# mlrun/mlrun

Measured on NVIDIA H100. Metric: events/sec, higher is better.
Workload: dtype f32 in / f64 accumulate

## Files before the change

mlrun_b200/csrc/b2s_rowthread.cuh:

```cuda
#pragma once
#include <cuda.h>
#include <type_traits>

#include "b2s_device.cuh"
#include "b2s_hash.cuh"

namespace b2s {

constexpr int kRTMaxCatCols = 16;
constexpr int kRTCatsInline = 4;
constexpr int kRTMaxCats = 256;

template <int NCH, int NS>
struct RTParams {
  const char* rows;
  int64_t row_stride;
  int64_t n_rows;
  float* out;
  int32_t* status;
  int32_t n_in, out_cols, n_models, vote_kind, out_is_int, fast_epilogue, tile_rows, pitch, stages, vec_ok;
  int32_t n_cat_cols, n_cat;
  int32_t one_sync;
  int32_t use_bulk;
  float* peers[8];
  int64_t peer_off;
  int32_t n_peers;
  MergeSig sig;
  const double* wcat;
  const double* vote_w_g;
  const ModelDesc* models;
  const int32_t* classes;
  double w[NCH * 4][NS];
  float fill[NCH * 4];
  float lim[NCH * 4];
  double bias[NS];
  double vote_w[NS];
  int32_t cat_col[kRTMaxCatCols];
  int32_t cat_off[kRTMaxCatCols];
  int32_t cat_sw[kRTMaxCatCols];
  int32_t cat_base[kRTMaxCatCols];
  int32_t cat_cnt[kRTMaxCatCols];
  float cat_fill[kRTMaxCatCols];
  float cat_inl[kRTMaxCatCols][kRTCatsInline];
  int32_t cat_first[kRTMaxCatCols];
  int32_t cat_dense[kRTMaxCatCols];
  float cat_val[kRTMaxCats];
  struct CatFast {
    int32_t off_b;
    int32_t sw_b;
    int32_t first;
    int32_t cnt;
    int32_t woff_b;
    float fill;
    int32_t pad[2];
  };
  CatFast catf[kRTMaxCatCols];
  int32_t cats_fast;
  int32_t zero_woff_b;
  int32_t dead_tail;
  int32_t pad_fast;
  const long long* g_keys;
  const TableSlot* g_slots;
  uint64_t g_mask;
  const float* g_values;
  long long g_missing_row;
};

struct RowPadded {
  const float* xr;
  __device__ __forceinline__ float4 chunk(int ch) const { return *reinterpret_cast<const float4*>(xr + ch * 4); }
  __device__ __forceinline__ float at2(int off, int) const { return xr[off]; }
  __device__ __forceinline__ float at_b(int off_b, int) const { return *reinterpret_cast<const float*>(reinterpret_cast<const char*>(xr) + off_b); }
};
struct RowSwizzled {
  const float* box0;
  int box_words;
  int r7s;
  __device__ __forceinline__ float4 chunk(int ch) const {
    return *reinterpret_cast<const float4*>(box0 + (ch >> 3) * box_words + (((ch & 7) << 2) ^ r7s));
  }
  __device__ __forceinline__ float at2(int off, int sw) const { return box0[off + (sw ^ r7s)]; }
  __device__ __forceinline__ float at_b(int off_b, int sw_b) const {
    return *reinterpret_cast<const float*>(reinterpret_cast<const char*>(box0) + off_b + (sw_b ^ (r7s << 2)));
  }
};

template <int NCH, int NS, int CH0, int CH1, typename Row>
__device__ __forceinline__ void rt_slice(const RTParams<NCH, NS>& p, const Row (&xr)[1], double (&acc)[1][NS]) {
  constexpr int RPT = 1;
  constexpr int BATCH = 4;
#pragma unroll
  for (int b = CH0; b < CH1; b += BATCH) {
    double xd[RPT][BATCH * 4];
#pragma unroll
    for (int cb = 0; cb < BATCH; ++cb) {
      const int ch = b + cb;
      if (ch < CH1) {
#pragma unroll
        for (int i = 0; i < RPT; ++i) {
          const float4 v = xr[i].chunk(ch);
          const float xs[4] = {v.x, v.y, v.z, v.w};
#pragma unroll
          for (int u = 0; u < 4; ++u) {
            const int c = ch * 4 + u;
            float x = xs[u];
            x = !(fabsf(x) <= p.lim[c]) ? p.fill[c] : x;
            xd[i][cb * 4 + u] = (double)x;
          }
        }
      }
    }
#pragma unroll
    for (int cb = 0; cb < BATCH; ++cb) {
      const int ch = b + cb;
      if (ch < CH1) {
#pragma unroll
        for (int u = 0; u < 4; ++u) {
          const int c = ch * 4 + u;
#pragma unroll
          for (int k = 0; k < NS; ++k)
#pragma unroll
            for (int i = 0; i < RPT; ++i) acc[i][k] = fma(p.w[c][k], xd[i][cb * 4 + u], acc[i][k]);
        }
      }
    }
  }
}

template <int NCH, int NS>
__device__ __noinline__ int rt_cat_search(const RTParams<NCH, NS>& p, int cc, float x) {
  const int b0 = p.cat_base[cc], cnt = p.cat_cnt[cc];
  int j = p.n_cat;
  if (cnt <= kRTCatsInline) {
#pragma unroll
    for (int qq = kRTCatsInline - 1; qq >= 0; --qq) j = (x == p.cat_inl[cc][qq]) ? b0 + qq : j;
  } else {
    for (int qq = cnt - 1; qq >= 0; --qq) j = (x == p.cat_val[b0 + qq]) ? b0 + qq : j;
  }
  return j;
}

template <int NCH, int NS, int Q0, int TPR, typename Row>
__device__ __forceinline__ void rt_cats(const RTParams<NCH, NS>& p, const Row (&xr)[1], const double* __restrict__ s_wcat,
                                        double (&acc)[1][NS]) {
  constexpr int RPT = 1;
  constexpr int ITERS = (kRTMaxCatCols - Q0 + TPR - 1) / TPR;
  if (p.cats_fast) {
    const char* wb = reinterpret_cast<const char*>(s_wcat);
#pragma unroll
    for (int it = 0; it < ITERS; ++it) {
      const int cc = Q0 + it * TPR;
      if (cc >= p.n_cat_cols) break;
      const typename RTParams<NCH, NS>::CatFast cf = p.catf[cc];
#pragma unroll
      for (int i = 0; i < RPT; ++i) {
        float x = xr[i].at_b(cf.off_b, cf.sw_b);
        x = (x != x) ? cf.fill : x;
        const int v = __float2int_rz(x);
        const unsigned jj = (unsigned)(v - cf.first);
        const bool miss = ((float)v != x) | (jj >= (unsigned)cf.cnt);
        const int a = miss ? p.zero_woff_b : cf.woff_b + (int)jj * (NS * 8);
        if constexpr (NS % 2 == 0) {
#pragma unroll
          for (int k = 0; k < NS; k += 2) {
            const double2 w2 = *reinterpret_cast<const double2*>(wb + a + k * 8);
            acc[i][k] += w2.x;
            acc[i][k + 1] += w2.y;
          }
        } else {
          const double* wc = reinterpret_cast<const double*>(wb + a);
#pragma unroll
          for (int k = 0; k < NS; ++k) acc[i][k] += wc[k];
        }
      }
    }
    return;
  }
#pragma unroll
  for (int it = 0; it < ITERS; ++it) {
    const int cc = Q0 + it * TPR;
    if (cc >= p.n_cat_cols) break;
#pragma unroll
    for (int i = 0; i < RPT; ++i) {
      float x = xr[i].at2(p.cat_off[cc], p.cat_sw[cc]);
      x = (x != x) ? p.cat_fill[cc] : x;
      int j;
      if (p.cat_dense[cc]) {
        const int v = __float2int_rz(x);
        const unsigned jj = (unsigned)(v - p.cat_first[cc]);
        j = ((float)v == x && jj < (unsigned)p.cat_cnt[cc]) ? p.cat_base[cc] + (int)jj : p.n_cat;
      } else {
        j = rt_cat_search(p, cc, x);
      }
      const double* wc = s_wcat + (size_t)j * NS;
#pragma unroll
      for (int k = 0; k < NS; ++k) acc[i][k] += wc[k];
    }
  }
}

template <int NCH, int NS, int TPR, int LIVE, typename Row>
__device__ __forceinline__ void rt_row_slices(const RTParams<NCH, NS>& p, int q, const Row (&xr)[1], const double* __restrict__ s_wcat,
                                              double (&acc)[1][NS]) {
  static_assert(LIVE % TPR == 0, "live chunks must split evenly over the row's threads");
  constexpr int CPT = LIVE / TPR;
  if (TPR == 1 || q == 0) {
    rt_slice<NCH, NS, 0, CPT>(p, xr, acc);
    rt_cats<NCH, NS, 0, TPR>(p, xr, s_wcat, acc);
  } else if (q == 1) {
    rt_slice<NCH, NS, (TPR > 1 ? CPT : 0), (TPR > 1 ? 2 * CPT : 0)>(p, xr, acc);
    rt_cats<NCH, NS, (TPR > 1 ? 1 : 0), TPR>(p, xr, s_wcat, acc);
  } else if (q == 2) {
    rt_slice<NCH, NS, (TPR > 2 ? 2 * CPT : 0), (TPR > 2 ? 3 * CPT : 0)>(p, xr, acc);
    rt_cats<NCH, NS, (TPR > 2 ? 2 : 0), TPR>(p, xr, s_wcat, acc);
  } else {
    rt_slice<NCH, NS, (TPR > 3 ? 3 * CPT : 0), (TPR > 3 ? 4 * CPT : 0)>(p, xr, acc);
    rt_cats<NCH, NS, (TPR > 3 ? 3 : 0), TPR>(p, xr, s_wcat, acc);
  }
}

__device__ __forceinline__ void mbar_init(uint64_t* bar, int count) {
  asm volatile("mbarrier.init.shared::cta.b64 [%0], %1;" ::"r"((uint32_t)__cvta_generic_to_shared(bar)), "r"(count));
}
__device__ __forceinline__ void mbar_expect_tx(uint64_t* bar, uint32_t bytes) {
  asm volatile("mbarrier.arrive.expect_tx.shared::cta.b64 _, [%0], %1;" ::"r"((uint32_t)__cvta_generic_to_shared(bar)), "r"(bytes)
               : "memory");
}
__device__ __forceinline__ void mbar_wait(uint64_t* bar, uint32_t parity) {
  const uint32_t a = (uint32_t)__cvta_generic_to_shared(bar);
  asm volatile(
      "{\n"
      ".reg .pred p;\n"
      "WAIT_%=:\n"
      "mbarrier.try_wait.parity.shared::cta.b64 p, [%0], %1;\n"
      "@p bra DONE_%=;\n"
      "bra WAIT_%=;\n"
      "DONE_%=:\n"
      "}\n" ::"r"(a), "r"(parity)
      : "memory");
}
__device__ __forceinline__ void bulk_load(void* smem_dst, const void* gsrc, uint32_t bytes, uint64_t* bar) {
  asm volatile("cp.async.bulk.shared::cluster.global.mbarrier::complete_tx::bytes [%0], [%1], %2, [%3];" ::"r"(
                   (uint32_t)__cvta_generic_to_shared(smem_dst)),
               "l"(gsrc), "r"(bytes), "r"((uint32_t)__cvta_generic_to_shared(bar))
               : "memory");
}

__device__ __forceinline__ void tensor_load_2d(void* smem_dst, const CUtensorMap* tmap, int x, int y, uint64_t* bar) {
  asm volatile(
      "cp.async.bulk.tensor.2d.shared::cluster.global.tile.mbarrier::complete_tx::bytes [%0], [%1, {%2, %3}], [%4];" ::"r"(
          (uint32_t)__cvta_generic_to_shared(smem_dst)),
      "l"(reinterpret_cast<uint64_t>(tmap)), "r"(x), "r"(y), "r"((uint32_t)__cvta_generic_to_shared(bar))
      : "memory");
}

template <int NCH, int NS>
__device__ __noinline__ void rt_generic_epilogue(const RTParams<NCH, NS>& p, const double* sl, int64_t row, uint32_t st) {
  double pred[kMaxModels];
  for (int m = 0; m < p.n_models; ++m) {
    const ModelDesc md = p.models[m];
    pred[m] = apply_link(md, sl + md.score_off, p.classes);
  }
  KParams kp;
  kp.out = p.out;
  kp.out_cols = p.out_cols;
  kp.n_models = p.n_models;
  kp.vote_kind = p.vote_kind;
  kp.out_is_int = p.out_is_int;
  kp.vote_w = p.vote_w_g;
  kp.status = p.status;
  kp.n_peers = p.n_peers;
  kp.peer_off = p.peer_off;
  for (int g = 0; g < p.n_peers; ++g) kp.peers[g] = p.peers[g];
  vote_and_store(kp, pred, row, st);
}

template <int NCH, int NS, int TPR, int LM>
__global__ void __launch_bounds__(128 * TPR, TPR >= 4 ? 2 : (TPR == 2 ? 3 : 4))
    rowthread_kernel(const __grid_constant__ RTParams<NCH, NS> p, const __grid_constant__ CUtensorMap tmap) {
  constexpr int RPT = 1;
  static_assert(NCH % TPR == 0, "chunks must split evenly over the row's threads");
  constexpr int CPT = NCH / TPR;
  extern __shared__ __align__(16) unsigned char smem[];
  uint64_t* s_bar = reinterpret_cast<uint64_t*>(smem);
  double* s_wcat = reinterpret_cast<double*>(smem + 64);
  const size_t wcat_bytes = 64 + (((size_t)(p.n_cat + 1) * NS * 8 + 15) / 16) * 16;
  const bool one_sync = (LM == 2) && TPR > 1 && p.one_sync;
  constexpr size_t part_words = (size_t)(TPR - 1) * 128 * NS;
  double* s_part = reinterpret_cast<double*>(smem + wcat_bytes);
  float* s_tiles = reinterpret_cast<float*>(smem + wcat_bytes + (one_sync ? 2 : 1) * part_words * 8);
  if (LM == 2) {
    const uint32_t a = (uint32_t)__cvta_generic_to_shared(s_tiles);
    s_tiles += ((1024u - (a & 1023u)) & 1023u) >> 2;
  }

  const int tid = threadIdx.x;
  const int TR = p.tile_rows;
  const int S = p.stages;
  const int tile_words = (LM == 2) ? TR * NCH * 4 : TR * p.pitch;
  const int64_t n_tiles = (p.n_rows + TR - 1) / TR;
  const int TRT = TR / RPT;
  const int q = tid / TRT;
  const int r = tid - q * TRT;

  const int cprv = p.vec_ok ? (p.n_in >> 2) : p.n_in;
  const int r0 = tid / cprv, c0 = tid - r0 * cprv;
  const int dr = (int)blockDim.x / cprv, dc = (int)blockDim.x - dr * cprv;
  auto issue = [&](float* tile, int64_t row0) {
    int64_t left = p.n_rows - row0;
    const int rows = left < TR ? (left < 0 ? 0 : (int)left) : TR;
    const char* base = p.rows + row0 * p.row_stride;
    int rr = r0, cc = c0;
    if (p.vec_ok) {
      while (rr < rows) {
        cp_async16(tile + rr * p.pitch + cc * 4, base + (int64_t)rr * p.row_stride + cc * 16);
        rr += dr;
        cc += dc;
        if (cc >= cprv) {
          cc -= cprv;
          ++rr;
        }
      }
    } else {
      while (rr < rows) {
        cp_async4(tile + rr * p.pitch + cc, base + (int64_t)rr * p.row_stride + cc * 4);
        rr += dr;
        cc += dc;
        if (cc >= cprv) {
          cc -= cprv;
          ++rr;
        }
      }
    }
  };

  constexpr bool bulk = LM != 0;
  const uint32_t row_bytes = (uint32_t)p.n_in * 4u;
  uint32_t unknown_bits = 0;
  long long gk_cur = 0, gk_nxt = 0;
  longlong2 g_slot = make_longlong2(0, -1);
  uint64_t g_hash = 0;
  int64_t g_tile_nxt = 0;
  auto g_key = [&](int64_t tile) -> long long {
    const int64_t row = tile * TR + tid;
    return row < p.n_rows ? __ldg(p.g_keys + row) : 0;
  };
  auto g_probe_start = [&](long long key) {
    g_hash = mix64((uint64_t)key) & p.g_mask;
    g_slot = __ldg(reinterpret_cast<const longlong2*>(p.g_slots) + g_hash);
  };
  auto g_probe_finish = [&](long long key) -> long long {
    uint64_t h = g_hash;
    longlong2 sl = g_slot;
    for (;;) {
      if (sl.y < 0) return -1;
      if (sl.x == key) return sl.y;
      h = (h + 1) & p.g_mask;
      sl = __ldg(reinterpret_cast<const longlong2*>(p.g_slots) + h);
    }
  };
  if (LM == 1 && p.g_keys && tid < TR) {
    gk_cur = g_key(blockIdx.x);
    gk_nxt = g_key((int64_t)blockIdx.x + gridDim.x);
    g_probe_start(gk_cur);
    g_tile_nxt = (int64_t)blockIdx.x + 2 * (int64_t)gridDim.x;
  }
  auto issue_bulk = [&](int st, int64_t row0) {
    int64_t left = p.n_rows - row0;
    const int rows = left < TR ? (left < 0 ? 0 : (int)left) : TR;
    if (LM == 2) {
      if (tid == 0) {
        if (rows > 0) {
          mbar_expect_tx(&s_bar[st], (uint32_t)(NCH / 8) * (uint32_t)TR * 128u);
#pragma unroll
          for (int b = 0; b < NCH / 8; ++b)
            tensor_load_2d(s_tiles + st * tile_words + b * TR * 32, &tmap, b * 32, (int)row0, &s_bar[st]);
        } else {
          mbar_expect_tx(&s_bar[st], 0);
        }
      }
    } else {
      if (tid == 0) mbar_expect_tx(&s_bar[st], (uint32_t)rows * row_bytes);
      if (p.g_keys) {
        if (tid < TR) {
          const long long hit = g_probe_finish(gk_cur);
          if (tid < rows) {
            unknown_bits = (unknown_bits & ~(1u << st)) | ((hit < 0 ? 1u : 0u) << st);
            bulk_load(s_tiles + st * tile_words + tid * p.pitch,
                      reinterpret_cast<const char*>(p.g_values + (hit < 0 ? p.g_missing_row : hit) * p.n_in), row_bytes, &s_bar[st]);
          }
          gk_cur = gk_nxt;
          g_probe_start(gk_cur);
          gk_nxt = g_key(g_tile_nxt);
          g_tile_nxt += gridDim.x;
        }
      } else if (tid < rows) {
        bulk_load(s_tiles + st * tile_words + tid * p.pitch, p.rows + (row0 + tid) * p.row_stride, row_bytes, &s_bar[st]);
      }
    }
  };
  if (bulk) {
    if (tid == 0) {
      for (int s = 0; s < S; ++s) mbar_init(&s_bar[s], 1);
      asm volatile("fence.mbarrier_init.release.cluster;" ::: "memory");
    }
    __syncthreads();
  }
  for (int s = 0; s < (one_sync ? S : S - 1); ++s) {
    const int64_t t = (int64_t)blockIdx.x + (int64_t)s * gridDim.x;
    if (bulk) {
      issue_bulk(s, t * TR);
    } else {
      if (t < n_tiles) issue(s_tiles + s * tile_words, t * TR);
      cp_async_commit();
    }
  }
  uint32_t phase_bits = 0;
  for (int i = tid; i < p.n_cat * NS; i += blockDim.x) s_wcat[i] = p.wcat[i];
  for (int i = tid; i < NS; i += blockDim.x) s_wcat[p.n_cat * NS + i] = 0.0;
  if (one_sync) __syncthreads();

  int stage = 0;
  uint32_t iter = 0;
  for (int64_t t = blockIdx.x; t < n_tiles; t += gridDim.x) {
    if (bulk) {
      mbar_wait(&s_bar[stage], (phase_bits >> stage) & 1u);
      phase_bits ^= (1u << stage);
    } else if (S == 2) cp_async_wait<0>();
    else if (S == 3) cp_async_wait<1>();
    else cp_async_wait<2>();
    if (!one_sync) {
      __syncthreads();
      const int64_t tn = t + (int64_t)(S - 1) * gridDim.x;
      int sn = stage + S - 1;
      if (sn >= S) sn -= S;
      if (bulk) {
        issue_bulk(sn, tn * TR);
      } else {
        if (tn < n_tiles) issue(s_tiles + sn * tile_words, tn * TR);
        cp_async_commit();
      }
    }
    const float* tile = s_tiles + stage * tile_words;
    const int64_t row0 = t * TR;
    const int live_rows = (int)(p.n_rows - row0 < (int64_t)TR ? p.n_rows - row0 : (int64_t)TR);
    const bool any_live = r < live_rows;
    using Row = typename std::conditional<LM == 2, RowSwizzled, RowPadded>::type;
    Row xr[RPT];
#pragma unroll
    for (int i = 0; i < RPT; ++i) {
      const int ri = r + i * TRT;
      if constexpr (LM == 2) {
        xr[i].box0 = tile + ri * 32;
        xr[i].box_words = TR * 32;
        xr[i].r7s = (r & 7) << 2;
      } else {
        xr[i].xr = tile + ri * p.pitch;
      }
    }
    double acc[RPT][NS];
#pragma unroll
    for (int i = 0; i < RPT; ++i)
#pragma unroll
      for (int k = 0; k < NS; ++k) acc[i][k] = 0.0;
    if (any_live) {
      if constexpr (LM == 2 && RPT == 1 && NCH >= 8 && (TPR == 1 || TPR == 2)) {
        if (p.dead_tail >= 4) rt_row_slices<NCH, NS, TPR, NCH - 4>(p, q, xr, s_wcat, acc);
        else if (p.dead_tail >= 2) rt_row_slices<NCH, NS, TPR, NCH - 2>(p, q, xr, s_wcat, acc);
        else rt_row_slices<NCH, NS, TPR, NCH>(p, q, xr, s_wcat, acc);
      } else {
        rt_row_slices<NCH, NS, TPR, NCH>(p, q, xr, s_wcat, acc);
      }
    }
    if (TPR > 1) {
      double* s_part_cur = s_part + (one_sync ? (size_t)(iter & 1) * part_words : 0);
      if (q > 0) {
#pragma unroll
        for (int i = 0; i < RPT; ++i) {
          double* part = s_part_cur + ((size_t)(q - 1) * 128 + r + i * TRT) * NS;
#pragma unroll
          for (int k = 0; k < NS; ++k) part[k] = acc[i][k];
        }
      }
      __syncthreads();
      if (one_sync) issue_bulk(stage, (t + (int64_t)S * gridDim.x) * TR);
      if (q == 0) {
#pragma unroll
        for (int i = 0; i < RPT; ++i)
#pragma unroll
          for (int qq = 1; qq < TPR; ++qq) {
            const double* o = s_part_cur + ((size_t)(qq - 1) * 128 + r + i * TRT) * NS;
#pragma unroll
            for (int k = 0; k < NS; ++k) acc[i][k] += o[k];
          }
      }
    }
#pragma unroll
    for (int i = 0; i < RPT; ++i) {
      const int64_t row = row0 + (r + i * TRT);
      if (q == 0 && r + i * TRT < live_rows) {
        uint32_t st = 0;
#pragma unroll
        for (int k = 0; k < NS; ++k) {
          acc[i][k] += p.bias[k];
          st |= (fabs(acc[i][k]) <= 1.7976931348623157e308) ? 0u : 1u;
        }
        if (LM == 1) st |= ((unknown_bits >> stage) & 1u) << 2;
        if (p.fast_epilogue) {
          if (p.vote_kind == 1) {
            double s = 0.0;
#pragma unroll
            for (int k = 0; k < NS; ++k) s = __dadd_rn(s, __dmul_rn(acc[i][k], p.vote_w[k]));
            store_word(p, row, 0, __float_as_uint((float)s));
          } else {
#pragma unroll
            for (int k = 0; k < NS; ++k)
              if (k < p.n_models) store_word(p, row, k, __float_as_uint((float)acc[i][k]));
          }
          if (p.status) p.status[row] = (int32_t)st;
        } else {
          double sl[NS];
#pragma unroll
          for (int k = 0; k < NS; ++k) sl[k] = acc[i][k];
          rt_generic_epilogue(p, sl, row, st);
        }
      }
    }
    ++stage;
    ++iter;
    if (stage == S) stage = 0;
  }
  cp_async_wait<0>();
  merge_signal(p.sig);
}

}
```

mlrun_b200/csrc/b2s_runtime.cu:

```cuda
#include <cuda_runtime.h>

#include <exception>

#include <algorithm>
#include <atomic>
#include <chrono>
#include <cmath>
#include <condition_variable>
#include <cstdarg>
#include <cstdio>
#include <cstdlib>
#include <cstring>
#include <deque>
#include <limits>
#include <map>
#include <memory>
#include <mutex>
#include <string>
#include <thread>
#include <vector>

#include "../../include/b200serve.h"
#include "b2s_internal.h"
#include "b2s_device.cuh"
// ... 181 lines not shown

int b2s_int_plan_shape(b2s_plan_s* p, int* n_in, int* out_cols) {
  if (!p || !p->finalized) return fail(B2S_ERR_STATE, "plan not finalized");
  *n_in = p->n_in;
  *out_cols = p->out_cols;
  return B2S_OK;
}

static size_t align_up(size_t x, size_t a) { return (x + a - 1) / a * a; }

struct BlobBuilder {
  std::vector<char> data;
  template <typename T>
  size_t add(const std::vector<T>& v) {
    size_t off = align_up(data.size(), 16);
    data.resize(off + std::max<size_t>(v.size() * sizeof(T), 16));
    if (!v.empty()) memcpy(data.data() + off, v.data(), v.size() * sizeof(T));
    return off;
  }
};

template <int MODE, int NS>
static cudaError_t launch_rows(const KParams& kp, int grid, int block, cudaStream_t st) {
  static std::atomic<bool> attr_set{false};
  if (!attr_set) {
    cudaError_t e = cudaFuncSetAttribute(rows_kernel<MODE, NS>, cudaFuncAttributeMaxDynamicSharedMemorySize,
                                         (int)G.prop.sharedMemPerBlockOptin);
    if (e != cudaSuccess) return e;
    attr_set = true;
  }
  rows_kernel<MODE, NS><<<grid, block, kp.sm_total, st>>>(kp);
  return cudaGetLastError();
}

static cudaError_t launch_plan(b2s_plan_s* p, const KParams& kp, int grid, int block, cudaStream_t st) {
  G.launches.fetch_add(1, std::memory_order_relaxed);
#define B2S_CASE(M, N) \
  if (p->mode == M && p->NS == N) return launch_rows<M, N>(kp, grid, block, st);
  B2S_CASE(MODE_LINEAR, 1) B2S_CASE(MODE_LINEAR, 2) B2S_CASE(MODE_LINEAR, 4) B2S_CASE(MODE_LINEAR, 8)
  B2S_CASE(MODE_LINEAR, 16) B2S_CASE(MODE_LINEAR, 32)
  B2S_CASE(MODE_TREES, 1) B2S_CASE(MODE_TREES, 4) B2S_CASE(MODE_TREES, 8) B2S_CASE(MODE_TREES, 16)
  B2S_CASE(MODE_TREES, 32) B2S_CASE(MODE_STORE, 1)
#undef B2S_CASE
  return cudaErrorInvalidValue;
}

typedef CUresult (*EncodeTiledFn)(CUtensorMap*, CUtensorMapDataType, cuuint32_t, void*, const cuuint64_t*, const cuuint64_t*,
                                  const cuuint32_t*, const cuuint32_t*, CUtensorMapInterleave, CUtensorMapSwizzle,
                                  CUtensorMapL2promotion, CUtensorMapFloatOOBfill);
static EncodeTiledFn tensor_map_encoder() {
  static EncodeTiledFn fn = [] {
    void* sym = nullptr;
    cudaDriverEntryPointQueryResult q;
    if (cudaGetDriverEntryPoint("cuTensorMapEncodeTiled", &sym, cudaEnableDefault, &q) != cudaSuccess || q != cudaDriverEntryPointSuccess) {
      cudaGetLastError();
      sym = nullptr;
    }
    return reinterpret_cast<EncodeTiledFn>(sym);
  }();
  return fn;
}
static bool encode_rows_map(CUtensorMap* map, const void* rows, int64_t n_rows, int64_t stride, int n_in, int tile_rows) {
  EncodeTiledFn enc = tensor_map_encoder();
  if (!enc) return false;
  cuuint64_t gdim[2] = {(cuuint64_t)n_in, (cuuint64_t)n_rows};
  cuuint64_t gstride[1] = {(cuuint64_t)stride};
  cuuint32_t box[2] = {32u, (cuuint32_t)tile_rows};
  cuuint32_t estr[2] = {1u, 1u};
  return enc(map, CU_TENSOR_MAP_DATA_TYPE_FLOAT32, 2, const_cast<void*>(rows), gdim, gstride, box, estr,
             CU_TENSOR_MAP_INTERLEAVE_NONE, CU_TENSOR_MAP_SWIZZLE_128B, CU_TENSOR_MAP_L2_PROMOTION_L2_128B,
             CU_TENSOR_MAP_FLOAT_OOB_FILL_NONE) == CUDA_SUCCESS;
}

struct RTTables {
  int n_in, n_out_cols, n_models, vote_kind, out_is_int, fast_epilogue, NS;
  const std::vector<float>* fill;
  const std::vector<uint32_t>* flags;
  const std::vector<double>* wnum;
  const std::vector<double>* bias;
  const std::vector<double>* vote_w;
  const std::vector<int32_t>* cat_off;
  const std::vector<float>* cat_val;
  const double* d_wcat;
  const double* d_vote_w;
  const ModelDesc* d_models;
  const int32_t* d_classes;
};

constexpr int rt_tpr(int NCH) { return NCH >= 8 ? 2 : 1; }
constexpr int kRTTileRows = 128, kRTStages = 2;

template <int NCH, int NS>
static void rt_build(b2s_plan_s* p, const RTTables& t) {
  using P = RTParams<NCH, NS>;
  p->rt_blob.assign(sizeof(P), 0);
  P& r = *reinterpret_cast<P*>(p->rt_blob.data());
  r.n_in = t.n_in;
  r.out_cols = t.n_out_cols;
  r.n_models = t.n_models;
  r.vote_kind = t.vote_kind;
  r.out_is_int = t.out_is_int;
  r.fast_epilogue = t.fast_epilogue;
  r.wcat = t.d_wcat;
  r.vote_w_g = t.d_vote_w;
  r.models = t.d_models;
  r.classes = t.d_classes;
  for (int c = 0; c < NCH * 4; ++c) {
    r.fill[c] = 0.0f;
    r.lim[c] = -1.0f;
    for (int k = 0; k < NS; ++k) r.w[c][k] = 0.0;
  }
  for (int c = 0; c < t.n_in; ++c) {
    const bool input = ((*t.flags)[c] & COL_COPIED) != 0;
    r.fill[c] = input ? (*t.fill)[c] : 0.0f;
    r.lim[c] = input ? std::numeric_limits<float>::infinity() : -1.0f;
    for (int k = 0; k < NS; ++k) r.w[c][k] = (*t.wnum)[(size_t)c * NS + k];
  }
  for (int k = 0; k < NS; ++k) {
    r.bias[k] = k < (int)t.bias->size() ? (*t.bias)[k] : 0.0;
    r.vote_w[k] = k < (int)t.vote_w->size() ? (*t.vote_w)[k] : 0.0;
  }
  int ncc = 0;
  for (int c = 0; c < t.n_in; ++c)
    if ((*t.cat_off)[c + 1] > (*t.cat_off)[c]) {
      r.cat_col[ncc] = c;
      r.cat_base[ncc] = (*t.cat_off)[c];
      r.cat_cnt[ncc] = (*t.cat_off)[c + 1] - (*t.cat_off)[c];
      r.cat_fill[ncc] = (*t.fill)[c];
      for (int q = 0; q < kRTCatsInline; ++q)
        r.cat_inl[ncc][q] = q < r.cat_cnt[ncc] ? (*t.cat_val)[r.cat_base[ncc] + q] : std::numeric_limits<float>::quiet_NaN();
      {
        const float f0 = (*t.cat_val)[r.cat_base[ncc]];
        bool dense = f0 == std::floor(f0) && std::fabs(f0) < 8388608.0f;
        for (int q = 0; dense && q < r.cat_cnt[ncc]; ++q) dense = (*t.cat_val)[r.cat_base[ncc] + q] == f0 + (float)q;
        r.cat_dense[ncc] = dense ? 1 : 0;
        r.cat_first[ncc] = dense ? (int)f0 : 0;
      }
      ++ncc;
    }
  r.n_cat_cols = ncc;
  r.n_cat = (int)t.cat_val->size();
  r.cats_fast = 1;
  for (int cc = 0; cc < ncc; ++cc) {
    r.cats_fast = r.cats_fast && r.cat_dense[cc];
    r.catf[cc].first = r.cat_first[cc];
    r.catf[cc].cnt = r.cat_cnt[cc];
    r.catf[cc].woff_b = r.cat_base[cc] * NS * 8;
    r.catf[cc].fill = r.cat_fill[cc];
  }
  r.zero_woff_b = r.n_cat * NS * 8;
  {
    int last_live = -1;
    for (int c = 0; c < t.n_in; ++c)
      if (((*t.flags)[c] & COL_COPIED) != 0) last_live = c >> 2;
    r.dead_tail = std::max(0, NCH - 1 - last_live);
    if (last_live < 0) r.dead_tail = 0;
  }
  for (int i = 0; i < r.n_cat; ++i) r.cat_val[i] = (*t.cat_val)[i];
}

struct LaunchCtx {
  const KParams* k = nullptr;
  bool host_rows = false;
};

template <int NCH, int NS>
static cudaError_t rt_launch_t(b2s_plan_s* p, const void* rows, int64_t stride, int64_t n_rows, void* out, int32_t* status,
                               int vec_ok, cudaStream_t st, bool query, int* occ, const B2SGather* gather, const LaunchCtx* lc) {
  using P = RTParams<NCH, NS>;
  constexpr int TPR = rt_tpr(NCH);
  constexpr int LMT = NCH >= 8 ? 2 : 1;
  static std::atomic<bool> attr_set{false};
  if (!attr_set) {
    const int cap = (int)G.prop.sharedMemPerBlockOptin;
    cudaError_t e = cudaFuncSetAttribute(rowthread_kernel<NCH, NS, TPR, 0>, cudaFuncAttributeMaxDynamicSharedMemorySize, cap);
    if (e == cudaSuccess) e = cudaFuncSetAttribute(rowthread_kernel<NCH, NS, TPR, 1>, cudaFuncAttributeMaxDynamicSharedMemorySize, cap);
    if (e == cudaSuccess && NCH >= 8)
      e = cudaFuncSetAttribute(rowthread_kernel<NCH, NS, TPR, LMT>, cudaFuncAttributeMaxDynamicSharedMemorySize, cap);
    if (e != cudaSuccess) return e;
    attr_set = true;
  }
  const bool tmap_ok = NCH >= 8 && p->n_in == NCH * 4 && tensor_map_encoder() != nullptr;
  if (query) {
    if (tmap_ok)
      return cudaOccupancyMaxActiveBlocksPerMultiprocessor(occ, rowthread_kernel<NCH, NS, TPR, LMT>, kRTTileRows * TPR, p->rt_smem);
    return cudaOccupancyMaxActiveBlocksPerMultiprocessor(occ, rowthread_kernel<NCH, NS, TPR, 0>, kRTTileRows * TPR, p->rt_smem);
  }
  P r = *reinterpret_cast<const P*>(p->rt_blob.data());
  r.rows = (const char*)rows;
  r.row_stride = stride;
  r.n_rows = n_rows;
  r.out = (float*)out;
  r.status = status;
  r.vec_ok = vec_ok;
  const KParams* lk = lc ? lc->k : nullptr;
  r.n_peers = lk ? lk->n_peers : (int)p->peers.size();
  r.peer_off = lk ? lk->peer_off : p->peer_off;
  for (int g = 0; g < r.n_peers; ++g) r.peers[g] = lk ? lk->peers[g] : (float*)p->peers[g];
  r.sig = lk ? lk->sig : MergeSig{};
  r.pitch = p->rt_pitch;
  r.stages = kRTStages;
  int mode = vec_ok ? 2 : 0;
  if (lc && lc->host_rows) mode = 0;
  if (mode == 2 && !tmap_ok) mode = 1;
  if (gather) {
    mode = 1;
    r.g_keys = gather->d_keys;
    r.g_slots = reinterpret_cast<const TableSlot*>(gather->d_slots);
    r.g_mask = gather->mask;
    r.g_values = gather->d_values;
    r.g_missing_row = gather->missing_row;
    if (gather->any_impute)
      for (int c = 0; c < p->n_in; ++c) {
        const float f = gather->h_impute[c];
        if (f == f && r.lim[c] == std::numeric_limits<float>::infinity()) {
          r.lim[c] = std::numeric_limits<float>::max();
          r.fill[c] = f;
        }
      }
  }
  int tr = kRTTileRows;
  while (tr > 32 && (n_rows + tr - 1) / tr < (int64_t)G.prop.multiProcessorCount) tr /= 2;
  alignas(64) CUtensorMap tmap;
  memset(&tmap, 0, sizeof(tmap));
  if (mode == 2 && !encode_rows_map(&tmap, rows, n_rows, stride, p->n_in, tr)) mode = 1;
  p->last_kernel.store(mode == 2 ? B2S_KERNEL_ROWTHREAD_TMA
                       : mode == 1 ? B2S_KERNEL_ROWTHREAD_BULK
                       : (lc && lc->host_rows) ? B2S_KERNEL_ROWTHREAD_HOST : B2S_KERNEL_ROWTHREAD_LDGSTS,
                       std::memory_order_relaxed);
  r.tile_rows = tr;
  const int64_t tiles = (n_rows + tr - 1) / tr;
  const int grid = (int)std::max<int64_t>(1, std::min<int64_t>(p->rt_grid, tiles));
  r.use_bulk = mode;
  r.one_sync = NS >= 4 ? 1 : 0;
  for (int cc = 0; cc < r.n_cat_cols; ++cc) {
    const int col = r.cat_col[cc], ch = col >> 2;
    r.cat_off[cc] = mode == 2 ? (ch >> 3) * (tr * 32) + (col & 3) : col;
    r.cat_sw[cc] = mode == 2 ? (ch & 7) << 2 : 0;
    r.catf[cc].off_b = r.cat_off[cc] * 4;
    r.catf[cc].sw_b = r.cat_sw[cc] * 4;
  }
  if (mode == 2)
    rowthread_kernel<NCH, NS, TPR, LMT><<<grid, tr * TPR, p->rt_smem, st>>>(r, tmap);
  else if (mode == 1)
    rowthread_kernel<NCH, NS, TPR, 1><<<grid, tr * TPR, p->rt_smem, st>>>(r, tmap);
  else
    rowthread_kernel<NCH, NS, TPR, 0><<<grid, tr * TPR, p->rt_smem, st>>>(r, tmap);
  return cudaGetLastError();
}

#define RT_DISPATCH(FN, ...)                                                              \
  do {                                                                                    \
    const int nch_ = p->rt_NCH, ns_ = p->rt_NS;                                           \
    if (nch_ == 4 && ns_ == 1) return FN<4, 1>(__VA_ARGS__);                              \
    if (nch_ == 4 && ns_ == 2) return FN<4, 2>(__VA_ARGS__);                              \
    if (nch_ == 4 && ns_ == 4) return FN<4, 4>(__VA_ARGS__);                              \
    if (nch_ == 4 && ns_ == 8) return FN<4, 8>(__VA_ARGS__);                              \
    if (nch_ == 8 && ns_ == 1) return FN<8, 1>(__VA_ARGS__);                              \
    if (nch_ == 8 && ns_ == 2) return FN<8, 2>(__VA_ARGS__);                              \
    if (nch_ == 8 && ns_ == 4) return FN<8, 4>(__VA_ARGS__);                              \
    if (nch_ == 8 && ns_ == 8) return FN<8, 8>(__VA_ARGS__);                              \
    if (nch_ == 16 && ns_ == 1) return FN<16, 1>(__VA_ARGS__);                            \
    if (nch_ == 16 && ns_ == 2) return FN<16, 2>(__VA_ARGS__);                            \
    if (nch_ == 16 && ns_ == 4) return FN<16, 4>(__VA_ARGS__);                            \
    if (nch_ == 16 && ns_ == 8) return FN<16, 8>(__VA_ARGS__);                            \
    if (nch_ == 32 && ns_ == 1) return FN<32, 1>(__VA_ARGS__);                            \
    if (nch_ == 32 && ns_ == 2) return FN<32, 2>(__VA_ARGS__);                            \
    if (nch_ == 32 && ns_ == 4) return FN<32, 4>(__VA_ARGS__);                            \
    if (nch_ == 32 && ns_ == 8) return FN<32, 8>(__VA_ARGS__);                            \
  } while (0)

static cudaError_t rt_launch(b2s_plan_s* p, const void* rows, int64_t stride, int64_t n_rows, void* out, int32_t* status,
                             int vec_ok, cudaStream_t st, bool query = false, int* occ = nullptr, const B2SGather* gather = nullptr,
                             const LaunchCtx* lc = nullptr) {
  RT_DISPATCH(rt_launch_t, p, rows, stride, n_rows, out, status, vec_ok, st, query, occ, gather, lc);
  return cudaErrorInvalidValue;
}
static void rt_build_any(b2s_plan_s* p, const RTTables& t) {
  RT_DISPATCH(rt_build, p, t);
}

extern "C" int b2s_version(void) { return B2S_VERSION; }
extern "C" const char* b2s_last_error(void) { return g_err.c_str(); }

extern "C" int b2s_init(int device_ordinal, const char* cfg) {
  try {
    std::lock_guard<std::mutex> lk(G.mu);
    if (G.inited) return B2S_OK;
    int n = 0;
    cudaError_t e = cudaGetDeviceCount(&n);
    if (e != cudaSuccess || n == 0)
      return fail(B2S_ERR_NO_DEVICE, "no CUDA device (%s); this engine has no CPU fallback",
                  e == cudaSuccess ? "device count 0" : cudaGetErrorString(e));
    if (device_ordinal < 0 || device_ordinal >= n) return fail(B2S_ERR_INVALID, "device ordinal %d out of range", device_ordinal);
    B2S_CUDA_TRY(cudaSetDevice(device_ordinal));
    B2S_CUDA_TRY(cudaGetDeviceProperties(&G.prop, device_ordinal));
    B2S_CUDA_TRY(cudaStreamCreateWithFlags(&G.stream, cudaStreamNonBlocking));
    B2S_CUDA_TRY(cudaStreamCreateWithFlags(&G.copy_stream, cudaStreamNonBlocking));
    G.device = device_ordinal;
    std::string c = cfg ? cfg : "";
    G.ring_slots = (int)cfg_get(c, "ring_slots", 4);
    G.max_batch = cfg_get(c, "max_batch", 65536);
    G.max_wait_us = cfg_get(c, "max_wait_us", 0);
    if (G.ring_slots < 2) G.ring_slots = 2;
    G.inited = true;
    return B2S_OK;
  } catch (const std::exception& e) {
    return fail(B2S_ERR_INVALID, "%s: %s", __func__, e.what());
  }
}

extern "C" int b2s_shutdown(void) {
  try {
    std::lock_guard<std::mutex> lk(G.mu);
    if (!G.inited) return B2S_OK;
    cudaStreamDestroy(G.stream);
    cudaStreamDestroy(G.copy_stream);
// ... 936 lines not shown
      block = tile_rows * tpr;
      stages = 3;
      blocks_per_sm = 2;
    } else if (p->mode == MODE_TREES) {
      block = 256;
      tile_rows = block / k.models_pow2;
      stages = 2;
      blocks_per_sm = 2;
    } else {
      block = 256;
      tile_rows = 128;
      stages = 2;
      blocks_per_sm = 2;
    }
    auto carve = [&](int tr, int st) {
      size_t off = 0;
      auto take = [&](size_t bytes) {
        size_t o = align_up(off, 16);
        off = o + bytes;
        return (int32_t)o;
      };
      k.sm_fill = take((size_t)n_in * 4);
      k.sm_flags = take((size_t)n_in * 4);
      k.sm_mapoff = take((size_t)(n_in + 1) * 4);
      k.sm_catoff = take((size_t)(n_in + 1) * 4);
      k.sm_catval = take(std::max<size_t>(cat_val.size(), 1) * 4);
      k.sm_wnum = take(p->mode == MODE_LINEAR ? (size_t)n_in * NS * 8 : 16);
      k.sm_wcat = take(p->mode == MODE_LINEAR ? std::max<size_t>(cat_val.size(), 1) * NS * 8 : 16);
      k.sm_outsrc = take((size_t)n_out * 4);
      k.sm_outkind = take((size_t)n_out * 4);
      k.sm_outarg = take((size_t)n_out * 4);
      k.sm_pred = take(p->mode == MODE_TREES ? (size_t)tr * k.models_pow2 * 8 : 16);
      k.sm_chunk = take((size_t)(n_in + 3) / 4 + 16);
      k.sm_part = take((p->mode == MODE_LINEAR && tpr > 1) ? (size_t)tr * tpr * NS * 8 : 16);
      k.sm_pst = take((p->mode == MODE_LINEAR && tpr > 1) ? (size_t)tr * tpr * 4 : 16);
      k.sm_exp = take((p->mode != MODE_LINEAR && need_expand) ? (size_t)tr * exp_pitch * 4 : 16);
      k.sm_tiles = take((size_t)st * tr * pitch * 4);
      return (int)align_up(off, 16);
    };
    int total = carve(tile_rows, stages);
    while (total * blocks_per_sm > smem_cap * 1 && (stages > 2 || blocks_per_sm > 1)) {
      if (stages > 2) --stages; else --blocks_per_sm;
      total = carve(tile_rows, stages);
    }
    while (total > smem_cap && stages > 1) total = carve(tile_rows, --stages);
    while (total > smem_cap && tile_rows > 8 && p->mode != MODE_LINEAR) {
      tile_rows /= 2;
      total = carve(tile_rows, stages);
    }
    if (total > smem_cap) {
      if (p->mode == MODE_LINEAR) {
        while (total > smem_cap && tile_rows > 8) {
          tile_rows /= 2;
          total = carve(tile_rows, stages);
        }
      }
      if (total > smem_cap) return fail(B2S_ERR_UNSUPPORTED, "plan needs %d B shared memory > %d B", total, smem_cap);
    }
    if (p->mode == MODE_TREES) block = std::max(32, tile_rows * k.models_pow2);
    if (p->mode == MODE_LINEAR) block = tile_rows * tpr;
    k.tpr = tpr;
    k.sm_total = total;
    k.tile_rows = tile_rows;
    k.pitch = pitch;
    k.exp_pitch = exp_pitch;
    k.stages = stages;
    p->NS = NS;
    p->block = block;
    int occ = std::max(1, std::min(blocks_per_sm, smem_cap / std::max(total, 1)));
    p->grid = sms * occ;

    {
      int n_cat_cols = 0;
      for (int c = 0; c < n_in; ++c) n_cat_cols += (cat_off[c + 1] > cat_off[c]) ? 1 : 0;
      if (p->mode == MODE_LINEAR && !any_map && n_in <= 128 && NS <= 8 && n_cat_cols <= kRTMaxCatCols &&
          (int)cat_val.size() <= kRTMaxCats) {
        const int nch = (n_in + 3) / 4;
        p->rt_NCH = nch <= 4 ? 4 : (nch <= 8 ? 8 : (nch <= 16 ? 16 : 32));
        p->rt_NS = NS;
        p->rt_cat_cols = n_cat_cols;
        bool simple = true;
        for (auto& m : p->models) simple = simple && m.link == B2S_LINK_IDENTITY && m.n_scores == 1;
        RTTables t{n_in, p->out_cols, M, p->vote_kind, p->out_is_int, (simple && p->vote_kind != B2S_VOTE_MAJORITY) ? 1 : 0, NS,
                   &p->fill, &flags, &wnum, &bias, &p->vote_w, &cat_off, &cat_val, k.wcat, k.vote_w, k.models, k.classes};
        rt_build_any(p, t);
        int rpitch = p->rt_NCH * 4 + 4;
        if (((rpitch / 4) & 1) == 0) rpitch += 4;
        p->rt_pitch = rpitch;
        {
          const size_t fixed = 1024 + 64 + align_up((size_t)(cat_val.size() + 1) * NS * 8, 16);
          const size_t part = (size_t)(rt_tpr(p->rt_NCH) - 1) * 128 * NS * 8;
          const size_t padded = fixed + part + (size_t)kRTStages * kRTTileRows * rpitch * 4;
          const size_t swizzled = fixed + 2 * part + (size_t)kRTStages * kRTTileRows * p->rt_NCH * 16;
          p->rt_smem = (int)std::max(padded, swizzled);
        }
        int occ = 0;
        if (p->rt_smem <= smem_cap && rt_launch(p, nullptr, 0, 0, nullptr, nullptr, 0, nullptr, true, &occ) == cudaSuccess && occ >= 1) {
          p->rt_ok = true;
          p->rt_grid = sms * occ;
        } else {
          cudaGetLastError();
        }
      }
    }
    if (p->mode == MODE_TREES && identity_schema && !any_map) {
      if (int rc = t3_build(p, k, any_fill)) return rc;
    }
    for (int i = 0; i < 4; ++i) B2S_CUDA_TRY(cudaEventCreate(&p->ev[i]));
    p->finalized = true;
    return B2S_OK;
  } catch (const std::exception& e) {
    return fail(B2S_ERR_INVALID, "%s: %s", __func__, e.what());
  }
}

extern "C" const char* b2s_plan_kernel(b2s_plan_t p) {
  if (!p || !p->finalized) return "";
  static thread_local char buf[200];
  const bool tmap = p->rt_NCH >= 8 && p->n_in == p->rt_NCH * 4 && tensor_map_encoder();
  if (p->dense_ok) snprintf(buf, sizeof(buf), "dense_head_kernel<N=%d> (wgmma tf32, %s, register accumulator groups; %d scores over %d columns)", p->dense.n_pad, p->dense.exact ? "exact 3-term input split" : "2-term input split", p->dense.n_scores, p->dense.n_in);
  else if (p->t3_ok) snprintf(buf, sizeof(buf), "t3_prep_kernel + trees3_kernel<D=%d,%s%s> + t3_vote_kernel (%d parts resident in shared memory, %d walking warps)", p->t3_D, p->t3_miss ? "NaN routing" : "floats", p->t3_cat ? ",categorical" : "", p->t3_parts, p->t3.warps);
  else if (p->rt_ok) snprintf(buf, sizeof(buf), "rowthread_kernel<NCH=%d,NS=%d,TPR=%d,%s>", p->rt_NCH, p->rt_NS, rt_tpr(p->rt_NCH), tmap ? "TMA tensor-map loads" : "TMA bulk loads");
  else snprintf(buf, sizeof(buf), "rows_kernel<%s,NS=%d>%s", p->mode == MODE_LINEAR ? "LINEAR" : (p->mode == MODE_TREES ? "TREES" : "STORE"), p->NS, p->any_cat ? " (categorical splits)" : "");
  return buf;
}

extern "C" int32_t b2s_plan_last_kernel(b2s_plan_t p) {
  return p ? p->last_kernel.load(std::memory_order_relaxed) : B2S_KERNEL_NONE;
}

extern "C" int b2s_plan_out_info(b2s_plan_t p, int32_t* out_cols, int32_t* out_is_int) {
  try {
    if (!p || !p->finalized) return fail(B2S_ERR_STATE, "plan not finalized");
    if (out_cols) *out_cols = p->out_cols;
    if (out_is_int) *out_is_int = p->out_is_int;
    return B2S_OK;
  } catch (const std::exception& e) {
    return fail(B2S_ERR_INVALID, "%s: %s", __func__, e.what());
  }
}

struct NvtxRange {
  explicit NvtxRange(const char* name) { nvtxRangePushA(name); }
  ~NvtxRange() { nvtxRangePop(); }
};

static int launch_on(b2s_plan_t p, const void* d_rows, int64_t n_rows, int64_t stride, void* d_out, int32_t* d_status,
                     cudaStream_t st, bool host_rows = false) {
  if (n_rows == 0) return B2S_OK;
  NvtxRange nvtx(p->dense_ok ? "b2s:dense_head" : p->t3_ok ? "b2s:trees3 (prep+walk+vote)"
                 : p->rt_ok ? "b2s:rowthread" : p->mode == MODE_STORE ? "b2s:rows_store" : "b2s:rows_kernel");
  KParams k = p->kp;
  k.rows = (const char*)d_rows;
  k.row_stride = stride;
  k.n_rows = n_rows;
  k.out = (float*)d_out;
  k.status = d_status;
  k.vec_ok = ((p->n_in % 4) == 0 && (stride % 16) == 0 && ((uintptr_t)d_rows % 16) == 0) ? 1 : 0;
  k.n_peers = (int)p->peers.size();
  k.peer_off = p->peer_off;
  for (int g = 0; g < k.n_peers; ++g) k.peers[g] = (float*)p->peers[g];
  k.sig = MergeSig{};
  if (p->comm) {
    b2s_comm_s* c = p->comm;
    if (n_rows > c->max_rows) return fail(B2S_ERR_INVALID, "shard of %lld rows exceeds the communicator's %lld", (long long)n_rows, (long long)c->max_rows);
    if (p->mode == MODE_STORE) return fail(B2S_ERR_UNSUPPORTED, "transform-only plans have no vote to merge");
    const uint32_t e = ++c->epoch;
    k.n_peers = c->world;
    k.peer_off = (int64_t)c->rank * c->max_rows;
    k.sig.n = c->world;
    k.sig.rank = c->rank;
    k.sig.epoch = e;
    k.sig.counter = c->counter();
    for (int g = 0; g < c->world; ++g) {
      const int r = (c->rank + 1 + g) % c->world;
      k.peers[g] = (float*)c->buf(r, e);
// ... 1009 lines not shown
```

Baseline: 10.46 billion.

## Compute numeric row dot products with FP64 DMMA tensor-core tiles

For NS>=2, the numeric-feature dot products move off per-thread FMA loops onto m16n8k4 FP64 mma.sync. One warp handles 32 rows with weights loaded from global memory, and the clamp limits and fill values are staged in shared memory. Results go to shared memory and are summed into the row owner's accumulators, while categorical features stay on the scalar path. The one-sync double-buffered partial scheme is removed, which adds a __syncthreads per tile and concentrates the work in a single warp per 32 rows, so parallelism across threads drops.

```diff
diff --git a/mlrun_b200/csrc/b2s_rowthread.cuh b/mlrun_b200/csrc/b2s_rowthread.cuh
--- a/mlrun_b200/csrc/b2s_rowthread.cuh
+++ b/mlrun_b200/csrc/b2s_rowthread.cuh
@@ -20,13 +20,13 @@
   int32_t* status;
   int32_t n_in, out_cols, n_models, vote_kind, out_is_int, fast_epilogue, tile_rows, pitch, stages, vec_ok;
   int32_t n_cat_cols, n_cat;
-  int32_t one_sync;
   int32_t use_bulk;
   float* peers[8];
   int64_t peer_off;
   int32_t n_peers;
   MergeSig sig;
   const double* wcat;
+  const double* wnum;
   const double* vote_w_g;
   const ModelDesc* models;
   const int32_t* classes;
@@ -127,6 +127,53 @@
   }
 }
 
+template <int NCH, int NS, int LIVE, int LM>
+__device__ __forceinline__ void rt_dmma_rows(const RTParams<NCH, NS>& p, const float* tile, int row0, const float2* __restrict__ s_lf,
+                                             double* __restrict__ s_dot) {
+  static_assert(NS >= 2 && NS <= 8 && NS % 2 == 0, "one n = 8 tile, score pairs per lane");
+  const int lane = threadIdx.x & 31, g = lane >> 2, t = lane & 3;
+  const float* xa;
+  int rstep, sw = 0, box_words = 0;
+  if constexpr (LM == 2) {
+    xa = tile + (row0 + g) * 32;
+    rstep = 8 * 32;
+    sw = ((g & 7) << 2) | t;
+    box_words = p.tile_rows * 32;
+  } else {
+    xa = tile + (row0 + g) * p.pitch + t;
+    rstep = 8 * p.pitch;
+  }
+  const int wlim = g < NS ? p.n_in : 0;
+  const double* wp = p.wnum + t * NS + g;
+  double d[2][4] = {};
+#pragma unroll
+  for (int ch = 0; ch < LIVE; ++ch) {
+    const int off = LM == 2 ? (ch >> 3) * box_words + (((ch & 7) << 2) ^ sw) : ch * 4;
+    const float2 lf = s_lf[ch * 4 + t];
+    const double b = (ch * 4 + t < wlim) ? __ldg(wp + ch * 4 * NS) : 0.0;
+    double a[4];
+#pragma unroll
+    for (int i = 0; i < 4; ++i) {
+      float x = xa[i * rstep + off];
+      x = !(fabsf(x) <= lf.x) ? lf.y : x;
+      a[i] = (double)x;
+    }
+#pragma unroll
+    for (int h = 0; h < 2; ++h)
+      asm("mma.sync.aligned.m16n8k4.row.col.f64.f64.f64.f64 {%0, %1, %2, %3}, {%4, %5}, {%6}, {%0, %1, %2, %3};"
+          : "+d"(d[h][0]), "+d"(d[h][1]), "+d"(d[h][2]), "+d"(d[h][3])
+          : "d"(a[2 * h]), "d"(a[2 * h + 1]), "d"(b));
+  }
+  if (2 * t < NS) {
+#pragma unroll
+    for (int h = 0; h < 2; ++h) {
+      double* o = s_dot + (size_t)(row0 + 16 * h + g) * NS + 2 * t;
+      *reinterpret_cast<double2*>(o) = make_double2(d[h][0], d[h][1]);
+      *reinterpret_cast<double2*>(o + 8 * NS) = make_double2(d[h][2], d[h][3]);
+    }
+  }
+}
+
 template <int NCH, int NS>
 __device__ __noinline__ int rt_cat_search(const RTParams<NCH, NS>& p, int cc, float x) {
   const int b0 = p.cat_base[cc], cnt = p.cat_cnt[cc];
@@ -285,10 +332,11 @@
   uint64_t* s_bar = reinterpret_cast<uint64_t*>(smem);
   double* s_wcat = reinterpret_cast<double*>(smem + 64);
   const size_t wcat_bytes = 64 + (((size_t)(p.n_cat + 1) * NS * 8 + 15) / 16) * 16;
-  const bool one_sync = (LM == 2) && TPR > 1 && p.one_sync;
-  constexpr size_t part_words = (size_t)(TPR - 1) * 128 * NS;
-  double* s_part = reinterpret_cast<double*>(smem + wcat_bytes);
-  float* s_tiles = reinterpret_cast<float*>(smem + wcat_bytes + (one_sync ? 2 : 1) * part_words * 8);
+  constexpr bool DMMA = NS >= 2;
+  constexpr size_t part_words = (size_t)(DMMA ? 1 : TPR - 1) * 128 * NS;
+  float2* s_lf = reinterpret_cast<float2*>(smem + wcat_bytes);
+  double* s_part = reinterpret_cast<double*>(smem + wcat_bytes + (DMMA ? NCH * 4 * 8 : 0));
+  float* s_tiles = reinterpret_cast<float*>(reinterpret_cast<unsigned char*>(s_part) + part_words * 8);
   if (LM == 2) {
     const uint32_t a = (uint32_t)__cvta_generic_to_shared(s_tiles);
     s_tiles += ((1024u - (a & 1023u)) & 1023u) >> 2;
@@ -406,7 +454,7 @@
     }
     __syncthreads();
   }
-  for (int s = 0; s < (one_sync ? S : S - 1); ++s) {
+  for (int s = 0; s < S - 1; ++s) {
     const int64_t t = (int64_t)blockIdx.x + (int64_t)s * gridDim.x;
     if (bulk) {
       issue_bulk(s, t * TR);
@@ -418,10 +466,10 @@
   uint32_t phase_bits = 0;
   for (int i = tid; i < p.n_cat * NS; i += blockDim.x) s_wcat[i] = p.wcat[i];
   for (int i = tid; i < NS; i += blockDim.x) s_wcat[p.n_cat * NS + i] = 0.0;
-  if (one_sync) __syncthreads();
+  if (DMMA)
+    for (int i = tid; i < NCH * 4; i += blockDim.x) s_lf[i] = make_float2(p.lim[i], p.fill[i]);
 
   int stage = 0;
-  uint32_t iter = 0;
   for (int64_t t = blockIdx.x; t < n_tiles; t += gridDim.x) {
     if (bulk) {
       mbar_wait(&s_bar[stage], (phase_bits >> stage) & 1u);
@@ -429,8 +477,8 @@
     } else if (S == 2) cp_async_wait<0>();
     else if (S == 3) cp_async_wait<1>();
     else cp_async_wait<2>();
-    if (!one_sync) {
-      __syncthreads();
+    __syncthreads();
+    {
       const int64_t tn = t + (int64_t)(S - 1) * gridDim.x;
       int sn = stage + S - 1;
       if (sn >= S) sn -= S;
@@ -463,7 +511,26 @@
     for (int i = 0; i < RPT; ++i)
 #pragma unroll
       for (int k = 0; k < NS; ++k) acc[i][k] = 0.0;
-    if (any_live) {
+    if constexpr (DMMA) {
+      if (q == 0 && any_live) rt_cats<NCH, NS, 0, 1>(p, xr, s_wcat, acc);
+      const int w0 = r & ~31;
+      if (q == TPR - 1 && w0 < live_rows) {
+        if constexpr (LM == 2 && NCH >= 8) {
+          if (p.dead_tail >= 4) rt_dmma_rows<NCH, NS, NCH - 4, LM>(p, tile, w0, s_lf, s_part);
+          else if (p.dead_tail >= 2) rt_dmma_rows<NCH, NS, NCH - 2, LM>(p, tile, w0, s_lf, s_part);
+          else rt_dmma_rows<NCH, NS, NCH, LM>(p, tile, w0, s_lf, s_part);
+        } else {
+          rt_dmma_rows<NCH, NS, NCH, LM>(p, tile, w0, s_lf, s_part);
+        }
+      }
+      if (TPR > 1) __syncthreads();
+      else __syncwarp();
+      if (q == 0) {
+        const double* o = s_part + (size_t)r * NS;
+#pragma unroll
+        for (int k = 0; k < NS; ++k) acc[0][k] += o[k];
+      }
+    } else if (any_live) {
       if constexpr (LM == 2 && RPT == 1 && NCH >= 8 && (TPR == 1 || TPR == 2)) {
         if (p.dead_tail >= 4) rt_row_slices<NCH, NS, TPR, NCH - 4>(p, q, xr, s_wcat, acc);
         else if (p.dead_tail >= 2) rt_row_slices<NCH, NS, TPR, NCH - 2>(p, q, xr, s_wcat, acc);
@@ -472,24 +539,22 @@
         rt_row_slices<NCH, NS, TPR, NCH>(p, q, xr, s_wcat, acc);
       }
     }
-    if (TPR > 1) {
-      double* s_part_cur = s_part + (one_sync ? (size_t)(iter & 1) * part_words : 0);
+    if (!DMMA && TPR > 1) {
       if (q > 0) {
 #pragma unroll
         for (int i = 0; i < RPT; ++i) {
-          double* part = s_part_cur + ((size_t)(q - 1) * 128 + r + i * TRT) * NS;
+          double* part = s_part + ((size_t)(q - 1) * 128 + r + i * TRT) * NS;
 #pragma unroll
           for (int k = 0; k < NS; ++k) part[k] = acc[i][k];
         }
       }
       __syncthreads();
-      if (one_sync) issue_bulk(stage, (t + (int64_t)S * gridDim.x) * TR);
       if (q == 0) {
 #pragma unroll
         for (int i = 0; i < RPT; ++i)
 #pragma unroll
           for (int qq = 1; qq < TPR; ++qq) {
-            const double* o = s_part_cur + ((size_t)(qq - 1) * 128 + r + i * TRT) * NS;
+            const double* o = s_part + ((size_t)(qq - 1) * 128 + r + i * TRT) * NS;
 #pragma unroll
             for (int k = 0; k < NS; ++k) acc[i][k] += o[k];
           }
@@ -527,7 +592,6 @@
       }
     }
     ++stage;
-    ++iter;
     if (stage == S) stage = 0;
   }
   cp_async_wait<0>();
diff --git a/mlrun_b200/csrc/b2s_runtime.cu b/mlrun_b200/csrc/b2s_runtime.cu
--- a/mlrun_b200/csrc/b2s_runtime.cu
+++ b/mlrun_b200/csrc/b2s_runtime.cu
@@ -287,6 +287,7 @@
   const std::vector<int32_t>* cat_off;
   const std::vector<float>* cat_val;
   const double* d_wcat;
+  const double* d_wnum;
   const double* d_vote_w;
   const ModelDesc* d_models;
   const int32_t* d_classes;
@@ -307,6 +308,7 @@
   r.out_is_int = t.out_is_int;
   r.fast_epilogue = t.fast_epilogue;
   r.wcat = t.d_wcat;
+  r.wnum = t.d_wnum;
   r.vote_w_g = t.d_vote_w;
   r.models = t.d_models;
   r.classes = t.d_classes;
@@ -437,7 +439,6 @@
   const int64_t tiles = (n_rows + tr - 1) / tr;
   const int grid = (int)std::max<int64_t>(1, std::min<int64_t>(p->rt_grid, tiles));
   r.use_bulk = mode;
-  r.one_sync = NS >= 4 ? 1 : 0;
   for (int cc = 0; cc < r.n_cat_cols; ++cc) {
     const int col = r.cat_col[cc], ch = col >> 2;
     r.cat_off[cc] = mode == 2 ? (ch >> 3) * (tr * 32) + (col & 3) : col;
@@ -1540,16 +1541,16 @@
         bool simple = true;
         for (auto& m : p->models) simple = simple && m.link == B2S_LINK_IDENTITY && m.n_scores == 1;
         RTTables t{n_in, p->out_cols, M, p->vote_kind, p->out_is_int, (simple && p->vote_kind != B2S_VOTE_MAJORITY) ? 1 : 0, NS,
-                   &p->fill, &flags, &wnum, &bias, &p->vote_w, &cat_off, &cat_val, k.wcat, k.vote_w, k.models, k.classes};
+                   &p->fill, &flags, &wnum, &bias, &p->vote_w, &cat_off, &cat_val, k.wcat, k.wnum, k.vote_w, k.models, k.classes};
         rt_build_any(p, t);
         int rpitch = p->rt_NCH * 4 + 4;
         if (((rpitch / 4) & 1) == 0) rpitch += 4;
         p->rt_pitch = rpitch;
         {
-          const size_t fixed = 1024 + 64 + align_up((size_t)(cat_val.size() + 1) * NS * 8, 16);
-          const size_t part = (size_t)(rt_tpr(p->rt_NCH) - 1) * 128 * NS * 8;
+          const size_t fixed = 1024 + 64 + align_up((size_t)(cat_val.size() + 1) * NS * 8, 16) + (NS >= 2 ? (size_t)p->rt_NCH * 32 : 0);
+          const size_t part = (size_t)(NS >= 2 ? 1 : rt_tpr(p->rt_NCH) - 1) * 128 * NS * 8;
           const size_t padded = fixed + part + (size_t)kRTStages * kRTTileRows * rpitch * 4;
-          const size_t swizzled = fixed + 2 * part + (size_t)kRTStages * kRTTileRows * p->rt_NCH * 16;
+          const size_t swizzled = fixed + part + (size_t)kRTStages * kRTTileRows * p->rt_NCH * 16;
           p->rt_smem = (int)std::max(padded, swizzled);
         }
         int occ = 0;
```

Result: faster. 10.75 billion, median of 6 (+2.8%).
